# tejeez/sxxcvr

Measured on NVIDIA B200. Metric: rx_unpack+tx_pack throughput, higher is better.
Workload: dtype s32<->f32

## Files before the change

sxxcvr_b200/csrc/sx_kernels.cuh:

```cuda
#pragma once

#include <cuda_runtime.h>
#include <stdint.h>

#include "sx_synth.h"

namespace sx {

template <int WORDS> struct Pack {
    uint32_t w[WORDS];
};

template <int BYTES> __device__ __forceinline__ Pack<BYTES / 4> ld_stream(const void *p);
template <int BYTES> __device__ __forceinline__ void st_stream(void *p, const Pack<BYTES / 4> &v);

template <> __device__ __forceinline__ Pack<1> ld_stream<4>(const void *p)
{
    Pack<1> r;
    asm volatile("ld.global.L1::no_allocate.b32 %0, [%1];" : "=r"(r.w[0]) : "l"(p) : "memory");
    return r;
}
template <> __device__ __forceinline__ Pack<2> ld_stream<8>(const void *p)
{
    Pack<2> r;
    asm volatile("ld.global.L1::no_allocate.v2.b32 {%0,%1}, [%2];"
                 : "=r"(r.w[0]), "=r"(r.w[1])
                 : "l"(p)
                 : "memory");
    return r;
}
template <> __device__ __forceinline__ Pack<4> ld_stream<16>(const void *p)
{
    Pack<4> r;
    asm volatile("ld.global.L1::no_allocate.v4.b32 {%0,%1,%2,%3}, [%4];"
                 : "=r"(r.w[0]), "=r"(r.w[1]), "=r"(r.w[2]), "=r"(r.w[3])
                 : "l"(p)
                 : "memory");
    return r;
}
template <> __device__ __forceinline__ Pack<8> ld_stream<32>(const void *p)
{
    Pack<8> r;
    asm volatile("ld.global.L1::no_allocate.L2::evict_first.v8.b32 {%0,%1,%2,%3,%4,%5,%6,%7}, [%8];"
                 : "=r"(r.w[0]), "=r"(r.w[1]), "=r"(r.w[2]), "=r"(r.w[3]), "=r"(r.w[4]),
                   "=r"(r.w[5]), "=r"(r.w[6]), "=r"(r.w[7])
                 : "l"(p)
                 : "memory");
    return r;
}

template <> __device__ __forceinline__ void st_stream<4>(void *p, const Pack<1> &v)
{
    asm volatile("st.global.L1::no_allocate.b32 [%0], %1;" ::"l"(p), "r"(v.w[0]) : "memory");
}
template <> __device__ __forceinline__ void st_stream<8>(void *p, const Pack<2> &v)
{
    asm volatile("st.global.L1::no_allocate.v2.b32 [%0], {%1,%2};" ::"l"(p), "r"(v.w[0]),
                 "r"(v.w[1])
                 : "memory");
}
template <> __device__ __forceinline__ void st_stream<16>(void *p, const Pack<4> &v)
{
    asm volatile("st.global.L1::no_allocate.v4.b32 [%0], {%1,%2,%3,%4};" ::"l"(p), "r"(v.w[0]),
                 "r"(v.w[1]), "r"(v.w[2]), "r"(v.w[3])
                 : "memory");
}
template <> __device__ __forceinline__ void st_stream<32>(void *p, const Pack<8> &v)
{
    asm volatile("st.global.L1::no_allocate.L2::evict_first.v8.b32 [%0], {%1,%2,%3,%4,%5,%6,%7,%8};" ::"l"(p),
                 "r"(v.w[0]), "r"(v.w[1]), "r"(v.w[2]), "r"(v.w[3]), "r"(v.w[4]), "r"(v.w[5]),
                 "r"(v.w[6]), "r"(v.w[7])
                 : "memory");
}


struct RxCf32 {
    static constexpr int kSrcWords = 2, kDstWords = 2;
    template <int FR>
    __device__ __forceinline__ static void apply(const Pack<2 * FR> &in, Pack<2 * FR> &out, float)
    {
#pragma unroll
        for (int i = 0; i < 2 * FR; i++)
            out.w[i] = __float_as_uint(__int2float_rn(int(in.w[i])) * 4.656612873077392578125e-10f);
    }
};

__device__ __forceinline__ uint32_t tx_component(float f)
{
    return uint32_t(__float2int_rz(f * 2147483648.0f)) & 0xFFFFFFFCu;
}

__device__ __forceinline__ uint32_t tx_enable_bits(float fi, float fq, float thr2)
{
    float mag2 = __fadd_rn(__fmul_rn(fi, fi), __fmul_rn(fq, fq));
    return (mag2 >= thr2) ? 3u : 0u;
}

struct TxCf32 {
    static constexpr int kSrcWords = 2, kDstWords = 2;
    template <int FR>
    __device__ __forceinline__ static void apply(const Pack<2 * FR> &in, Pack<2 * FR> &out,
                                                 float thr2)
    {
#pragma unroll
        for (int n = 0; n < FR; n++) {
            float fi = __uint_as_float(in.w[2 * n]), fq = __uint_as_float(in.w[2 * n + 1]);
            out.w[2 * n] = tx_component(fi) | tx_enable_bits(fi, fq, thr2);
            out.w[2 * n + 1] = tx_component(fq);
        }
    }
};

struct RxCs16 {
    static constexpr int kSrcWords = 2, kDstWords = 1;
    template <int FR>
    __device__ __forceinline__ static void apply(const Pack<2 * FR> &in, Pack<FR> &out, float)
    {
#pragma unroll
        for (int n = 0; n < FR; n++)
            out.w[n] = __byte_perm(in.w[2 * n], in.w[2 * n + 1], 0x7632);
    }
};

struct TxCs16 {
    static constexpr int kSrcWords = 1, kDstWords = 2;
    template <int FR>
    __device__ __forceinline__ static void apply(const Pack<FR> &in, Pack<2 * FR> &out, float thr2)
    {
#pragma unroll
        for (int n = 0; n < FR; n++) {
            uint32_t w = in.w[n];
            float fi = __int2float_rn(int(short(w & 0xFFFFu))) * 3.0517578125e-05f;
            float fq = __int2float_rn(int(w) >> 16) * 3.0517578125e-05f;
            out.w[2 * n] = (w << 16) | tx_enable_bits(fi, fq, thr2);
            out.w[2 * n + 1] = w & 0xFFFF0000u;
        }
    }
};

struct RxS16Cf32 {
    static constexpr int kSrcWords = 1, kDstWords = 2;
    template <int FR>
    __device__ __forceinline__ static void apply(const Pack<FR> &in, Pack<2 * FR> &out, float)
    {
#pragma unroll
        for (int n = 0; n < FR; n++) {
            uint32_t w = in.w[n];
            out.w[2 * n] = __float_as_uint(__int2float_rn(int(short(w & 0xFFFFu))) * 3.0517578125e-05f);
            out.w[2 * n + 1] = __float_as_uint(__int2float_rn(int(w) >> 16) * 3.0517578125e-05f);
        }
    }
};

struct TxCf32S16 {
    static constexpr int kSrcWords = 2, kDstWords = 1;
    __device__ __forceinline__ static uint32_t component(float f)
    {
        int v = __float2int_rz(f * 32768.0f);
        v = v > 32767 ? 32767 : (v < -32768 ? -32768 : v);
        return uint32_t(v) & 0xFFFCu;
    }
    template <int FR>
    __device__ __forceinline__ static void apply(const Pack<2 * FR> &in, Pack<FR> &out, float thr2)
    {
#pragma unroll
        for (int n = 0; n < FR; n++) {
            float fi = __uint_as_float(in.w[2 * n]), fq = __uint_as_float(in.w[2 * n + 1]);
            out.w[n] = (component(fi) | tx_enable_bits(fi, fq, thr2)) | (component(fq) << 16);
        }
    }
};

struct StreamArgs {
    const char *src;
    char *dst;
    uint64_t total;
    uint64_t head;
    uint64_t nvec;
    float thr2;
};

template <class Op, int FR, int UNROLL, int BLOCK>
__global__ void __launch_bounds__(BLOCK) stream_convert_kernel(const StreamArgs a)
{
    constexpr int SB = Op::kSrcWords * 4 * FR, DB = Op::kDstWords * 4 * FR;
    constexpr uint64_t TILE = uint64_t(BLOCK) * UNROLL;
    const char *src = a.src + a.head * (Op::kSrcWords * 4);
    char *dst = a.dst + a.head * (Op::kDstWords * 4);

    for (uint64_t base = uint64_t(blockIdx.x) * TILE; base < a.nvec;
         base += uint64_t(gridDim.x) * TILE) {
        Pack<Op::kSrcWords * FR> in[UNROLL];
        Pack<Op::kDstWords * FR> out[UNROLL];
        const uint64_t first = base + threadIdx.x;
        const char *sp = src + first * SB;
        char *dp = dst + first * DB;
        if (base + TILE <= a.nvec) {
#pragma unroll
            for (int j = 0; j < UNROLL; j++)
                in[j] = ld_stream<SB>(sp + size_t(j) * BLOCK * SB);
#pragma unroll
            for (int j = 0; j < UNROLL; j++)
                Op::template apply<FR>(in[j], out[j], a.thr2);
#pragma unroll
            for (int j = 0; j < UNROLL; j++)
                st_stream<DB>(dp + size_t(j) * BLOCK * DB, out[j]);
        } else {
#pragma unroll
            for (int j = 0; j < UNROLL; j++) {
                if (first + uint64_t(j) * BLOCK < a.nvec) {
                    in[j] = ld_stream<SB>(sp + size_t(j) * BLOCK * SB);
                    Op::template apply<FR>(in[j], out[j], a.thr2);
                    st_stream<DB>(dp + size_t(j) * BLOCK * DB, out[j]);
                }
            }
        }
    }

    if (blockIdx.x == 0) {
        const uint64_t mid = a.nvec * FR;
        const uint64_t nedge = a.total - mid;
        if (threadIdx.x < nedge) {
            uint64_t f = threadIdx.x < a.head ? threadIdx.x : mid + threadIdx.x;
            Pack<Op::kSrcWords> in1 = ld_stream<Op::kSrcWords * 4>(a.src + f * (Op::kSrcWords * 4));
            Pack<Op::kDstWords> out1;
            Op::template apply<1>(in1, out1, a.thr2);
            st_stream<Op::kDstWords * 4>(a.dst + f * (Op::kDstWords * 4), out1);
        }
    }
}

template <class Op>
__global__ void word_convert_kernel(const char *src, char *dst, uint64_t total, float thr2)
{
    for (uint64_t f = uint64_t(blockIdx.x) * blockDim.x + threadIdx.x; f < total;
         f += uint64_t(gridDim.x) * blockDim.x) {
        Pack<Op::kSrcWords> in;
        Pack<Op::kDstWords> out;
#pragma unroll
        for (int i = 0; i < Op::kSrcWords; i++)
            in.w[i] = ld_stream<4>(src + (f * Op::kSrcWords + i) * 4).w[0];
        Op::template apply<1>(in, out, thr2);
#pragma unroll
        for (int i = 0; i < Op::kDstWords; i++) {
            Pack<1> o;
            o.w[0] = out.w[i];
            st_stream<4>(dst + (f * Op::kDstWords + i) * 4, o);
        }
    }
}

namespace bulk {

__device__ __forceinline__ uint32_t smem_u32(const void *p)
{
    return uint32_t(__cvta_generic_to_shared(p));
}
__device__ __forceinline__ void mbar_init(uint64_t *bar, uint32_t count)
{
    asm volatile("mbarrier.init.shared::cta.b64 [%0], %1;" ::"r"(smem_u32(bar)), "r"(count));
}
__device__ __forceinline__ void mbar_expect_tx(uint64_t *bar, uint32_t bytes)
{
    asm volatile("mbarrier.arrive.expect_tx.shared::cta.b64 _, [%0], %1;" ::"r"(smem_u32(bar)),
                 "r"(bytes)
                 : "memory");
}
__device__ __forceinline__ void mbar_wait(uint64_t *bar, uint32_t parity)
{
    asm volatile("{\n"
                 ".reg .pred p;\n"
                 "WAIT_%=:\n"
                 "mbarrier.try_wait.parity.shared::cta.b64 p, [%0], %1;\n"
                 "@p bra DONE_%=;\n"
                 "bra WAIT_%=;\n"
                 "DONE_%=:\n"
                 "}" ::"r"(smem_u32(bar)),
                 "r"(parity)
                 : "memory");
}
__device__ __forceinline__ uint64_t make_policy(int kind)
{
    uint64_t pol;
    switch (kind) {
    case 1: asm volatile("createpolicy.fractional.L2::evict_normal.b64 %0, 1.0;" : "=l"(pol)); break;
    case 2: asm volatile("createpolicy.fractional.L2::evict_last.b64 %0, 1.0;" : "=l"(pol)); break;
    case 3: asm volatile("createpolicy.fractional.L2::evict_unchanged.b64 %0, 1.0;" : "=l"(pol)); break;
    default: asm volatile("createpolicy.fractional.L2::evict_first.b64 %0, 1.0;" : "=l"(pol)); break;
    }
    return pol;
}
__device__ __forceinline__ void load_g2s(void *smem_dst, const void *gsrc, uint32_t bytes,
                                         uint64_t *bar, uint64_t pol)
{
    asm volatile("cp.async.bulk.shared::cluster.global.mbarrier::complete_tx::bytes.L2::cache_hint "
                 "[%0], [%1], %2, [%3], %4;" ::"r"(smem_u32(smem_dst)),
                 "l"(gsrc), "r"(bytes), "r"(smem_u32(bar)), "l"(pol)
                 : "memory");
}
__device__ __forceinline__ void store_s2g(void *gdst, const void *smem_src, uint32_t bytes,
                                          uint64_t pol)
{
    asm volatile("cp.async.bulk.global.shared::cta.bulk_group.L2::cache_hint [%0], [%1], %2, %3;" ::"l"(gdst),
                 "r"(smem_u32(smem_src)), "r"(bytes), "l"(pol)
                 : "memory");
}
__device__ __forceinline__ void commit_group()
{
    asm volatile("cp.async.bulk.commit_group;" ::: "memory");
}
template <int N> __device__ __forceinline__ void wait_group_read()
{
    asm volatile("cp.async.bulk.wait_group.read %0;" ::"n"(N) : "memory");
}
__device__ __forceinline__ void wait_group_all()
{
    asm volatile("cp.async.bulk.wait_group 0;" ::: "memory");
}
__device__ __forceinline__ void fence_async_smem()
{
    asm volatile("fence.proxy.async.shared::cta;" ::: "memory");
}

}

struct BulkArgs {
    const char *src;
    char *dst;
    uint64_t nframes;
    float thr2;
    int load_policy;
    int store_policy;
    int contiguous;
};

template <class Op, int TILE, int STAGES, bool SKEW = false>
__global__ void bulk_convert_kernel(const BulkArgs a)
{
    constexpr int SFB = Op::kSrcWords * 4, DFB = Op::kDstWords * 4;
    static_assert(!SKEW || (SFB == 8 && DFB == 8), "the skewed variant is for 8-byte frames on both sides");
    constexpr int PAD = SKEW ? 16 : 0;
    constexpr size_t IN_STAGE = size_t(TILE) * SFB + PAD;
    extern __shared__ __align__(128) unsigned char smem[];
    unsigned char *in_buf = smem;
    unsigned char *out_buf = smem + size_t(STAGES) * IN_STAGE;
    uint64_t *full = reinterpret_cast<uint64_t *>(out_buf + size_t(STAGES) * TILE * DFB);

    const uint64_t ntiles = (a.nframes + TILE - 1) / TILE;
    uint64_t first, stride, mine;
    if (a.contiguous) {
        const uint64_t per = (ntiles + gridDim.x - 1) / gridDim.x;
        first = uint64_t(blockIdx.x) * per;
        stride = 1;
        mine = first >= ntiles ? 0 : (ntiles - first < per ? ntiles - first : per);
    } else {
        first = blockIdx.x;
        stride = gridDim.x;
        mine = first >= ntiles ? 0 : (ntiles - first + stride - 1) / stride;
    }
    if (mine == 0)
        return;
    const uint64_t pol = bulk::make_policy(a.load_policy), pol_store = bulk::make_policy(a.store_policy);

    auto tile_frames = [&](uint64_t i) -> uint32_t {
        uint64_t t = first + i * stride;
        uint64_t left = a.nframes - t * TILE;
        return uint32_t(left < uint64_t(TILE) ? left : uint64_t(TILE));
    };

    if (threadIdx.x == 0) {
        for (int s = 0; s < STAGES; s++)
            bulk::mbar_init(&full[s], 1);
        asm volatile("fence.mbarrier_init.release.cluster;" ::: "memory");
    }
    __syncthreads();

    if (threadIdx.x == 0) {
        for (uint64_t i = 0; i < uint64_t(STAGES) && i < mine; i++) {
            uint32_t nf = tile_frames(i);
            bulk::mbar_expect_tx(&full[i], nf * SFB + PAD);
            bulk::load_g2s(in_buf + i * IN_STAGE, a.src + (first + i * stride) * TILE * SFB,
                           nf * SFB + PAD, &full[i], pol);
        }
    }

    for (uint64_t i = 0; i < mine; i++) {
        const int s = int(i % STAGES);
        const uint32_t parity = uint32_t(i / STAGES) & 1u;
        const uint32_t nf = tile_frames(i);

        if (threadIdx.x == 0)
            bulk::wait_group_read<STAGES - 1>();
        __syncthreads();

        bulk::mbar_wait(&full[s], parity);

        const unsigned char *ib = in_buf + size_t(s) * IN_STAGE + (SKEW ? 8 : 0);
        unsigned char *ob = out_buf + size_t(s) * TILE * DFB;
        constexpr int FR = (Op::kSrcWords == 1 || Op::kDstWords == 1) ? 4 : 2;
        for (uint32_t v = threadIdx.x; v * FR < nf; v += blockDim.x) {
            Pack<Op::kSrcWords * FR> in;
            Pack<Op::kDstWords * FR> out;
            if constexpr (SKEW) {
                const uint2 *ip = reinterpret_cast<const uint2 *>(ib + size_t(v) * FR * SFB);
#pragma unroll
                for (int q = 0; q < FR; q++) {
                    uint2 t = ip[q];
                    in.w[2 * q] = t.x, in.w[2 * q + 1] = t.y;
                }
            } else {
                const uint4 *ip = reinterpret_cast<const uint4 *>(ib + size_t(v) * FR * SFB);
#pragma unroll
                for (int q = 0; q < Op::kSrcWords * FR / 4; q++) {
                    uint4 t = ip[q];
                    in.w[4 * q] = t.x, in.w[4 * q + 1] = t.y, in.w[4 * q + 2] = t.z, in.w[4 * q + 3] = t.w;
                }
            }
            Op::template apply<FR>(in, out, a.thr2);
            uint4 *op = reinterpret_cast<uint4 *>(ob + size_t(v) * FR * DFB);
#pragma unroll
            for (int q = 0; q < Op::kDstWords * FR / 4; q++)
                op[q] = make_uint4(out.w[4 * q], out.w[4 * q + 1], out.w[4 * q + 2], out.w[4 * q + 3]);
        }
        bulk::fence_async_smem();
        __syncthreads();

        if (threadIdx.x == 0) {
            bulk::store_s2g(a.dst + (first + i * stride) * TILE * DFB, ob, nf * DFB, pol_store);
            bulk::commit_group();
            uint64_t nxt = i + STAGES;
            if (nxt < mine) {
                uint32_t nnf = tile_frames(nxt);
                bulk::mbar_expect_tx(&full[s], nnf * SFB + PAD);
                bulk::load_g2s(in_buf + size_t(s) * IN_STAGE,
                               a.src + (first + nxt * stride) * TILE * SFB, nnf * SFB + PAD, &full[s], pol);
            }
        }
    }
    if (threadIdx.x == 0)
        bulk::wait_group_all();
}

struct LoopbackArgs {
    const char *i2s_in;
    char *cf32;
    char *i2s_out;
    uint64_t nvec;
    uint64_t total;
    float thr2;
};

template <int UNROLL>
__global__ void loopback_kernel(const LoopbackArgs a)
{
    const uint64_t tile = uint64_t(blockDim.x) * UNROLL;
    for (uint64_t base = uint64_t(blockIdx.x) * tile; base < a.nvec;
         base += uint64_t(gridDim.x) * tile) {
        Pack<4> in[UNROLL];
#pragma unroll
        for (int j = 0; j < UNROLL; j++) {
            uint64_t v = base + threadIdx.x + uint64_t(j) * blockDim.x;
            if (v < a.nvec)
                in[j] = ld_stream<16>(a.i2s_in + v * 16);
        }
#pragma unroll
        for (int j = 0; j < UNROLL; j++) {
            uint64_t v = base + threadIdx.x + uint64_t(j) * blockDim.x;
            if (v < a.nvec) {
                Pack<4> mid, out;
                RxCf32::apply<2>(in[j], mid, 0.0f);
                TxCf32::apply<2>(mid, out, a.thr2);
                if (a.cf32)
                    st_stream<16>(a.cf32 + v * 16, mid);
                st_stream<16>(a.i2s_out + v * 16, out);
            }
        }
    }
    if (blockIdx.x == 0 && threadIdx.x == 0 && (a.total & 1)) {
        uint64_t f = a.total - 1;
        Pack<2> in1 = ld_stream<8>(a.i2s_in + f * 8), mid, out;
        RxCf32::apply<1>(in1, mid, 0.0f);
        TxCf32::apply<1>(mid, out, a.thr2);
        if (a.cf32)
            st_stream<8>(a.cf32 + f * 8, mid);
        st_stream<8>(a.i2s_out + f * 8, out);
    }
}

struct BlockDesc {
    const char *src;
    char *dst;
    uint64_t length;
    float thr2;
    uint32_t reserved;
};

template <class Op>
__device__ __forceinline__ void convert_span(const BlockDesc &b, uint64_t lo, uint64_t hi,
                                             uint32_t tid, uint32_t nthreads)
{
    constexpr int SFB = Op::kSrcWords * 4, DFB = Op::kDstWords * 4;
    constexpr int FR = 16 / (SFB < DFB ? SFB : DFB);
    const bool vec_ok = ((reinterpret_cast<uintptr_t>(b.src) + lo * SFB) % (SFB * FR) == 0) &&
                        ((reinterpret_cast<uintptr_t>(b.dst) + lo * DFB) % (DFB * FR) == 0);
    uint64_t done = lo;
    if (vec_ok) {
        uint64_t nvec = (hi - lo) / FR;
        constexpr int U = 4;
        uint64_t v = tid;
        for (; v + uint64_t(U - 1) * nthreads < nvec; v += uint64_t(U) * nthreads) {
            Pack<Op::kSrcWords * FR> in[U];
#pragma unroll
            for (int u = 0; u < U; u++)
                in[u] = ld_stream<SFB * FR>(b.src + (lo + (v + uint64_t(u) * nthreads) * FR) * SFB);
#pragma unroll
            for (int u = 0; u < U; u++) {
// ... 505 lines not shown
```

sxxcvr_b200/csrc/sxgpu.cu:

```cuda
#include "../../include/sxgpu.h"

#include "sx_kernels.cuh"
#include "sx_bank.cuh"
#include "sx_iir.cuh"
#include "sx_resident.cuh"
#include "host/par_copy.hpp"
#include "host/worker_pool.hpp"

#include <algorithm>
#include <atomic>
#include <chrono>
#include <cmath>
#include <cstdio>
#include <cstdlib>
#include <cstring>
#include <map>
#include <memory>
#include <mutex>
#include <string>
#include <tuple>
#include <type_traits>
#include <vector>

#include <sched.h>

using namespace sx;

namespace {

constexpr int kRingSlots = 4;

struct HostRing {
    size_t chunk_frames = 0;
    void *d_in[kRingSlots] = {};
    void *d_out[kRingSlots] = {};
    void *h_in[kRingSlots] = {};
    void *h_out[kRingSlots] = {};
    cudaEvent_t copied_in[kRingSlots] = {};
    cudaEvent_t converted[kRingSlots] = {};
    cudaEvent_t done[kRingSlots] = {};
    bool events = false;
};

struct alignas(64) SmallFlag {
    volatile unsigned long long done;
};

struct HostLane {
    std::mutex mutex;
    cudaStream_t s_h2d = nullptr, s_comp = nullptr, s_d2h = nullptr;
    cudaStream_t s_slot[kRingSlots] = {};
    HostRing ring;
    std::unique_ptr<sxhost::ParallelCopier> copier_in, copier_out;
    sxhost::Sidekick retirer;
    sxhost::Progress issued, retired;
    std::atomic<int> pipeline_error{0};

    SmallFlag *flag = nullptr;
    unsigned int *d_arrivals = nullptr;
    unsigned long long flag_seq = 0;

    Mailbox *mailbox = nullptr;
    cudaStream_t s_resident = nullptr;
    unsigned long long resident_seq = 0;
};

}

struct sxgpu_ctx {
    int device = 0;
    cudaDeviceProp prop;
    cudaStream_t stream = nullptr;

    int64_t rx_variant = 0, tx_variant = 0;
    int64_t unroll = 0;
    int64_t block = 0;
    int64_t ctas_per_sm = 0;
    int64_t bulk_tile = 0, bulk_stages = 0;
    int64_t bulk_load_policy = 0, bulk_store_policy = 0;
    int64_t bulk_contiguous = 0;
    int64_t host_chunk_frames = 0;
    int64_t host_chunk_min_frames = 0;
    int64_t host_mode = 0;
    int64_t small_mode = 0;
    int64_t host_in_mode = 0;
    int64_t host_out_mode = 0;
    int64_t bounce_nt = 1;
    int64_t pipeline_mode = 0;
    int64_t zero_copy_max_frames = 1 << 18;
    int64_t resident_max_frames = 0;
    int64_t zero_copy_variant = 1;
    int64_t batch_variant = 0;
    int64_t loopback_variant = 0;
    int64_t warp_ctas_per_sm = 0;
    int64_t bank_split_variant = 0;
    int64_t bank_pdl = 1;
    int64_t bank_repeat_variant = 0;
    int64_t bounce_threads = 0;
    int64_t numa_local_alloc = 1;
    int64_t numa_node = -1;

    cpu_set_t local_cpus;
    bool have_local_cpus = false;

    std::atomic<uint64_t> resident_launches{0}, resident_calls{0}, flagged_calls{0};
    std::atomic<int> live_banks{0};
    std::atomic<int> live_iirs{0};
    bool l2_carveout_set = false;

    HostLane lanes[2];

    cudaMemPool_t scratch_pool = nullptr;

    StatsAcc *d_stats = nullptr;
    StatsAcc *h_stats = nullptr;
    std::mutex stats_mutex;

    std::atomic<uint64_t> launches{0}, frames_rx{0}, frames_tx{0}, h2d_bytes{0}, d2h_bytes{0};

    std::mutex err_mutex;
    std::string last_error;
    uint64_t error_serial = 0;

    std::mutex occupancy_mutex;
    std::map<std::tuple<const void *, int, size_t>, int> occupancy;

    int fail(cudaError_t e, const char *what)
    {
        std::lock_guard<std::mutex> lock(err_mutex);
        last_error = std::string(what) + ": " + cudaGetErrorString(e);
        error_serial++;
        cudaGetLastError();
        return (e == cudaErrorMemoryAllocation) ? SXGPU_ERR_NOMEM : SXGPU_ERR_CUDA;
    }
    int invalid(const char *what)
    {
        std::lock_guard<std::mutex> lock(err_mutex);
        last_error = what;
        error_serial++;
        return SXGPU_ERR_INVALID;
    }
};

namespace {

void read_gpu_locality(sxgpu_ctx *ctx)
{
    CPU_ZERO(&ctx->local_cpus);
    char bdf[32] = {0};
    if (cudaDeviceGetPCIBusId(bdf, sizeof bdf, ctx->device) != cudaSuccess) {
        cudaGetLastError();
        return;
    }
    for (char *c = bdf; *c; c++)
        if (*c >= 'A' && *c <= 'F')
            *c = char(*c - 'A' + 'a');
    const std::string base = std::string("/sys/bus/pci/devices/") + bdf + "/";
    if (FILE *f = std::fopen((base + "numa_node").c_str(), "r")) {
        long node = -1;
        if (std::fscanf(f, "%ld", &node) == 1)
            ctx->numa_node = node;
        std::fclose(f);
    }
    if (FILE *f = std::fopen((base + "local_cpulist").c_str(), "r")) {
        int lo = 0, hi = 0, count = 0;
        for (;;) {
            if (std::fscanf(f, "%d", &lo) != 1)
                break;
            hi = lo;
            int c = std::fgetc(f);
            if (c == '-') {
                if (std::fscanf(f, "%d", &hi) != 1)
                    break;
                c = std::fgetc(f);
            }
            for (int cpu = lo; cpu <= hi && cpu < CPU_SETSIZE; cpu++, count++)
                CPU_SET(cpu, &ctx->local_cpus);
            if (c != ',')
                break;
        }
        std::fclose(f);
        ctx->have_local_cpus = count > 0;
    }
}

class NearGpu {
public:
    explicit NearGpu(sxgpu_ctx *ctx)
    {
        if (!ctx->numa_local_alloc || !ctx->have_local_cpus)
            return;
        if (sched_getaffinity(0, sizeof saved_, &saved_) != 0)
            return;
        cpu_set_t want;
        CPU_AND(&want, &saved_, &ctx->local_cpus);
        if (CPU_COUNT(&want) == 0 || CPU_EQUAL(&want, &saved_))
            return;
        bound_ = sched_setaffinity(0, sizeof want, &want) == 0;
    }
    ~NearGpu()
    {
        if (bound_)
            sched_setaffinity(0, sizeof saved_, &saved_);
    }
    NearGpu(const NearGpu &) = delete;
    NearGpu &operator=(const NearGpu &) = delete;

private:
    cpu_set_t saved_;
    bool bound_ = false;
};

}

#define SX_CUDA(ctx, call)                                                                     \
    do {                                                                                       \
        cudaError_t e_ = (call);                                                               \
        if (e_ != cudaSuccess)                                                                 \
            return (ctx)->fail(e_, #call);                                                     \
    } while (0)

#define SX_TRY(expr)                                                                           \
    do {                                                                                       \
        int r_ = (expr);                                                                       \
        if (r_ != SXGPU_OK)                                                                    \
            return r_;                                                                         \
    } while (0)

namespace {

typedef void (*StreamKernel)(const StreamArgs);
typedef void (*BulkKernel)(const BulkArgs);

template <class Op, int FR, int BLOCK> StreamKernel stream_kernel_for_unroll(int unroll)
{
    switch (unroll) {
    case 2: return stream_convert_kernel<Op, FR, 2, BLOCK>;
    case 8: return stream_convert_kernel<Op, FR, 8, BLOCK>;
    default: return stream_convert_kernel<Op, FR, 4, BLOCK>;
    }
}

template <class Op> StreamKernel stream_kernel(int fr, int unroll, int block)
{
    if (fr == 4)
        return block == 512 ? stream_kernel_for_unroll<Op, 4, 512>(unroll)
                            : stream_kernel_for_unroll<Op, 4, 256>(unroll);
    if (fr == 2)
        return block == 512 ? stream_kernel_for_unroll<Op, 2, 512>(unroll)
                            : stream_kernel_for_unroll<Op, 2, 256>(unroll);
    return stream_convert_kernel<Op, 1, 4, 256>;
}

struct BulkShape {
    int tile, stages;
};

template <class Op> BulkKernel bulk_kernel(BulkShape s)
{
    if (s.tile == 4096 && s.stages == 3) return bulk_convert_kernel<Op, 4096, 3>;
    if (s.tile == 3072 && s.stages == 4) return bulk_convert_kernel<Op, 3072, 4>;
    if (s.tile == 2048 && s.stages == 6) return bulk_convert_kernel<Op, 2048, 6>;
    if (s.tile == 2048 && s.stages == 5) return bulk_convert_kernel<Op, 2048, 5>;
    if (s.tile == 2048 && s.stages == 4) return bulk_convert_kernel<Op, 2048, 4>;
    if (s.tile == 2048 && s.stages == 3) return bulk_convert_kernel<Op, 2048, 3>;
    if (s.tile == 1024 && s.stages == 6) return bulk_convert_kernel<Op, 1024, 6>;
    if (s.tile == 1024 && s.stages == 4) return bulk_convert_kernel<Op, 1024, 4>;
    if (s.tile == 512 && s.stages == 4) return bulk_convert_kernel<Op, 512, 4>;
    return nullptr;
}

template <class Op> size_t bulk_smem_bytes(BulkShape s, bool skew = false)
{
    return size_t(s.stages) * (size_t(s.tile) * (Op::kSrcWords + Op::kDstWords) * 4 + (skew ? 16 : 0)) +
           size_t(s.stages) * 8;
}

template <class Op> BulkKernel bulk_skew_kernel(BulkShape s)
{
    if constexpr (Op::kSrcWords == 2 && Op::kDstWords == 2) {
        if (s.tile == 2048 && s.stages == 4) return bulk_convert_kernel<Op, 2048, 4, true>;
        if (s.tile == 1024 && s.stages == 4) return bulk_convert_kernel<Op, 1024, 4, true>;
    }
    return nullptr;
}

int normalise_unroll(int64_t u)
{
    return (u == 2 || u == 4 || u == 8) ? int(u) : 4;
}

template <class K>
int persistent_grid(sxgpu_ctx *ctx, K kernel, int block, size_t smem, uint64_t work_items)
{
    int per_sm = int(ctx->ctas_per_sm);
    if (per_sm <= 0) {
        std::lock_guard<std::mutex> lock(ctx->occupancy_mutex);
        auto key = std::make_tuple(reinterpret_cast<const void *>(kernel), block, smem);
        auto it = ctx->occupancy.find(key);
        if (it == ctx->occupancy.end()) {
            int occ = 0;
            if (cudaOccupancyMaxActiveBlocksPerMultiprocessor(&occ, kernel, block, smem) != cudaSuccess ||
                occ <= 0) {
                cudaGetLastError();
                occ = 1;
            }
            it = ctx->occupancy.emplace(key, occ).first;
        }
        per_sm = it->second;
    }
    uint64_t grid = uint64_t(ctx->prop.multiProcessorCount) * uint64_t(per_sm);
    grid = std::min<uint64_t>(grid, std::max<uint64_t>(work_items, 1));
    return int(grid);
}

struct Plan {
    int fr = 0;
    uint64_t head = 0;
};

template <class Op> Plan plan_access(const char *src, const char *dst, uint64_t total, int want_fr)
{
    constexpr uintptr_t SFB = Op::kSrcWords * 4, DFB = Op::kDstWords * 4;
    uintptr_t s = reinterpret_cast<uintptr_t>(src), d = reinterpret_cast<uintptr_t>(dst);
    Plan p;
    if (s % SFB != 0 || d % DFB != 0)
        return p;
    for (int fr = want_fr; fr >= 1; fr >>= 1) {
        uintptr_t a = (s / SFB) % fr, b = (d / DFB) % fr;
        if (a != b)
            continue;
        p.fr = fr;
        p.head = std::min<uint64_t>((fr - a) % fr, total);
        return p;
    }
    p.fr = 1;
    return p;
}

template <class Op>
int launch_bulk(sxgpu_ctx *ctx, const char *src, const char *dst_c, uint64_t total, float thr2,
                cudaStream_t st, bool *handled)
{
    char *dst = const_cast<char *>(dst_c);
    constexpr uintptr_t SFB = Op::kSrcWords * 4, DFB = Op::kDstWords * 4;
    constexpr uint64_t G = 16 / (SFB < DFB ? SFB : DFB);
    *handled = false;

    uint64_t head = 0;
    bool found = false;
    for (; head < G; head++) {
        if ((reinterpret_cast<uintptr_t>(src) + head * SFB) % 16 == 0 &&
            (reinterpret_cast<uintptr_t>(dst) + head * DFB) % 16 == 0) {
            found = true;
            break;
        }
    }

    const int big_tile = (SFB == DFB) ? 2048 : 3072;
    BulkShape shape = {int(ctx->bulk_tile ? ctx->bulk_tile : (total >= (uint64_t(1) << 24) ? big_tile : 1024)),
                       int(ctx->bulk_stages ? ctx->bulk_stages : 4)};
    BulkKernel k = nullptr;
    bool skew = false;
    uint64_t mid = 0;
    if (found) {
        if (total < head + G)
            return SXGPU_OK;
        mid = (total - head) / G * G;
        k = bulk_kernel<Op>(shape);
        if (!k)
            return ctx->invalid("unsupported bulk_tile/bulk_stages combination");
    } else {
        k = bulk_skew_kernel<Op>(shape);
        if (!k || reinterpret_cast<uintptr_t>(src) % 8 || reinterpret_cast<uintptr_t>(dst) % 8)
            return SXGPU_OK;
        head = (reinterpret_cast<uintptr_t>(dst) % 16) ? 1 : 2;
        if (total < head + 3)
            return SXGPU_OK;
        mid = (total - head - 1) / 2 * 2;
        skew = true;
    }
    size_t smem = bulk_smem_bytes<Op>(shape, skew);
    int block = int(ctx->block ? ctx->block : 256);

    BulkArgs a = {src + head * SFB - (skew ? 8 : 0), dst + head * DFB, mid, thr2, int(ctx->bulk_load_policy),
                  int(ctx->bulk_store_policy), int(ctx->bulk_contiguous)};
    uint64_t ntiles = (mid + shape.tile - 1) / shape.tile;
    int grid = persistent_grid(ctx, k, block, smem, ntiles);
    k<<<grid, block, smem, st>>>(a);
    SX_CUDA(ctx, cudaGetLastError());
    ctx->launches++;

    uint64_t tail = total - head - mid;
    if (head) {
        StreamArgs e = {src, dst, head, head, 0, thr2};
        stream_convert_kernel<Op, 1, 4, 256><<<1, 256, 0, st>>>(e);
        SX_CUDA(ctx, cudaGetLastError());
        ctx->launches++;
    }
    if (tail) {
        StreamArgs e = {src + (head + mid) * SFB, dst + (head + mid) * DFB, tail, tail, 0, thr2};
        stream_convert_kernel<Op, 1, 4, 256><<<1, 256, 0, st>>>(e);
        SX_CUDA(ctx, cudaGetLastError());
        ctx->launches++;
    }
    *handled = true;
    return SXGPU_OK;
}

template <class Op>
int launch_convert(sxgpu_ctx *ctx, const void *src_v, void *dst_v, uint64_t total, float thr2,
                   int64_t variant, cudaStream_t st)
{
    if (total == 0)
        return SXGPU_OK;
    const char *src = static_cast<const char *>(src_v);
    char *dst = static_cast<char *>(dst_v);
    if (reinterpret_cast<uintptr_t>(src) % 4 || reinterpret_cast<uintptr_t>(dst) % 4)
        return ctx->invalid("sample buffers must be at least 4-byte aligned");

    if (variant == 0)
        variant = 4;
    if (variant == 4) {
        constexpr bool narrow = Op::kSrcWords != Op::kDstWords;
        Plan p = plan_access<Op>(src, dst, total, narrow ? 4 : 2);
        if (p.fr >= 2 && total >= p.head + uint64_t(p.fr)) {
            constexpr int block = 256;
            const int unroll = total < (uint64_t(1) << 21) ? 4 : 2;
            StreamArgs a = {src, dst, total, p.head, (total - p.head) / uint64_t(p.fr), thr2};
            StreamKernel k = stream_kernel<Op>(p.fr, unroll, block);
            uint64_t tiles = (a.nvec + uint64_t(block) * unroll - 1) / (uint64_t(block) * unroll);
            k<<<unsigned(std::min<uint64_t>(tiles, 0x7fffffffu)), block, 0, st>>>(a);
            SX_CUDA(ctx, cudaGetLastError());
            ctx->launches++;
            return SXGPU_OK;
        }
        variant = 3;
    }
    if (variant == 3) {
        bool handled = false;
        SX_TRY(launch_bulk<Op>(ctx, src, dst, total, thr2, st, &handled));
        if (handled)
            return SXGPU_OK;
        variant = 1;
    }

    Plan p = plan_access<Op>(src, dst, total, variant == 2 ? 4 : 2);
    if (p.fr == 0) {
        const int block = 256;
        uint64_t ctas = (total + block - 1) / block;
        int grid = persistent_grid(ctx, word_convert_kernel<Op>, block, 0, ctas);
        word_convert_kernel<Op><<<grid, block, 0, st>>>(src, dst, total, thr2);
        SX_CUDA(ctx, cudaGetLastError());
        ctx->launches++;
        return SXGPU_OK;
    }

    int unroll = p.fr == 1 ? 4 : normalise_unroll(ctx->unroll);
    int block = (p.fr != 1 && ctx->block == 512) ? 512 : 256;
    StreamArgs a = {src, dst, total, p.head, (total - p.head) / uint64_t(p.fr), thr2};
    StreamKernel k = stream_kernel<Op>(p.fr, unroll, block);
    uint64_t tiles = (a.nvec + uint64_t(block) * unroll - 1) / (uint64_t(block) * unroll);
    int grid = persistent_grid(ctx, k, block, 0, tiles);
    k<<<grid, block, 0, st>>>(a);
    SX_CUDA(ctx, cudaGetLastError());
    ctx->launches++;
    return SXGPU_OK;
}

bool frames_overflow(size_t offset, size_t length)
{
    const size_t cap = size_t(1) << 60;
    return offset > cap || length > cap || offset + length > cap;
}

template <class Op>
int convert_entry(sxgpu_ctx *ctx, const void *d_src, size_t src_offset, void *d_dest,
                  size_t dest_offset, size_t length, float thr2, int64_t variant,
                  sxgpu_stream stream)
{
    if (!ctx)
        return SXGPU_ERR_INVALID;
    if (length == 0)
        return SXGPU_OK;
    if (!d_src || !d_dest)
        return ctx->invalid("null sample buffer");
    if (frames_overflow(src_offset, length) || frames_overflow(dest_offset, length))
        return ctx->invalid("offset + length overflows");
    SX_CUDA(ctx, cudaSetDevice(ctx->device));
    const char *src = static_cast<const char *>(d_src) + src_offset * (Op::kSrcWords * 4);
    char *dst = static_cast<char *>(d_dest) + dest_offset * (Op::kDstWords * 4);
    cudaStream_t st = stream ? static_cast<cudaStream_t>(stream) : ctx->stream;
    return launch_convert<Op>(ctx, src, dst, length, thr2, variant, st);
}

struct HostPtrInfo {
    bool pinned = false;
    bool on_device = false;
    bool foreign_device = false;
    void *device_alias = nullptr;
};

HostPtrInfo classify_pointer(const sxgpu_ctx *ctx, const void *p)
{
    HostPtrInfo info;
    cudaPointerAttributes attr;
    if (cudaPointerGetAttributes(&attr, p) != cudaSuccess) {
        cudaGetLastError();
        return info;
    }
    if (attr.type == cudaMemoryTypeHost) {
        info.pinned = true;
        info.device_alias = attr.devicePointer;
    } else if (attr.type == cudaMemoryTypeDevice || attr.type == cudaMemoryTypeManaged) {
        info.on_device = true;
        info.foreign_device = attr.type == cudaMemoryTypeDevice && attr.device != ctx->device;
        info.device_alias = attr.devicePointer;
    }
    return info;
}

size_t pick_chunk_frames(const sxgpu_ctx *ctx, size_t length)
{
    if (ctx->host_chunk_frames > 0)
        return size_t(std::max<int64_t>(ctx->host_chunk_frames, 1024));
    size_t chunk = size_t(1) << 17;
    while (chunk < (size_t(1) << 22) && chunk * 4 < length)
        chunk <<= 1;
    return chunk;
}

int ensure_lane(sxgpu_ctx *ctx, HostLane &lane)
{
    if (!lane.s_h2d) {
        SX_CUDA(ctx, cudaStreamCreateWithFlags(&lane.s_h2d, cudaStreamDefault));
        SX_CUDA(ctx, cudaStreamCreateWithFlags(&lane.s_comp, cudaStreamDefault));
        SX_CUDA(ctx, cudaStreamCreateWithFlags(&lane.s_d2h, cudaStreamDefault));
        for (int i = 0; i < kRingSlots; i++)
            SX_CUDA(ctx, cudaStreamCreateWithFlags(&lane.s_slot[i], cudaStreamDefault));
    }
    HostRing &r = lane.ring;
    if (!r.events) {
        for (int i = 0; i < kRingSlots; i++) {
            SX_CUDA(ctx, cudaEventCreateWithFlags(&r.copied_in[i], cudaEventDisableTiming));
            SX_CUDA(ctx, cudaEventCreateWithFlags(&r.converted[i], cudaEventDisableTiming));
            SX_CUDA(ctx, cudaEventCreateWithFlags(&r.done[i], cudaEventDisableTiming));
        }
        r.events = true;
    }
    if (!lane.flag) {
        SX_CUDA(ctx, cudaHostAlloc(reinterpret_cast<void **>(&lane.flag), sizeof(SmallFlag),
                                   cudaHostAllocMapped | cudaHostAllocPortable));
        lane.flag->done = 0;
        SX_CUDA(ctx, cudaMalloc(reinterpret_cast<void **>(&lane.d_arrivals), sizeof(unsigned int)));
        SX_CUDA(ctx, cudaMemset(lane.d_arrivals, 0, sizeof(unsigned int)));
    }
    return SXGPU_OK;
}

void resident_stop(sxgpu_ctx *, HostLane &lane)
{
    if (!lane.mailbox || !lane.s_resident)
        return;
    volatile Mailbox *box = lane.mailbox;
    box->quit = 1;
    std::atomic_thread_fence(std::memory_order_seq_cst);
    cudaStreamSynchronize(lane.s_resident);
    box->quit = 0;
}

int ensure_ring(sxgpu_ctx *ctx, HostLane &lane, size_t frames, bool bounce_in, bool bounce_out)
{
    SX_TRY(ensure_lane(ctx, lane));
    HostRing &r = lane.ring;
    if (frames > r.chunk_frames) {
        resident_stop(ctx, lane);
        for (int i = 0; i < kRingSlots; i++) {
            if (r.d_in[i]) cudaFree(r.d_in[i]);
            if (r.d_out[i]) cudaFree(r.d_out[i]);
            if (r.h_in[i]) cudaFreeHost(r.h_in[i]);
            if (r.h_out[i]) cudaFreeHost(r.h_out[i]);
            r.d_in[i] = r.d_out[i] = r.h_in[i] = r.h_out[i] = nullptr;
        }
        r.chunk_frames = 0;
        for (int i = 0; i < kRingSlots; i++) {
            SX_CUDA(ctx, cudaMalloc(&r.d_in[i], frames * 8));
            SX_CUDA(ctx, cudaMalloc(&r.d_out[i], frames * 8));
        }
        r.chunk_frames = frames;
    }
    bool missing = false;
    for (int i = 0; i < kRingSlots; i++)
        missing = missing || (bounce_in && !r.h_in[i]) || (bounce_out && !r.h_out[i]);
    if (!missing)
        return SXGPU_OK;
    NearGpu near(ctx);
    for (int i = 0; i < kRingSlots; i++) {
        if (bounce_in && !r.h_in[i])
            SX_CUDA(ctx, cudaHostAlloc(&r.h_in[i], r.chunk_frames * 8, cudaHostAllocDefault));
        if (bounce_out && !r.h_out[i])
            SX_CUDA(ctx, cudaHostAlloc(&r.h_out[i], r.chunk_frames * 8, cudaHostAllocDefault));
    }
    return SXGPU_OK;
}

int resident_convert_call(sxgpu_ctx *ctx, HostLane &lane, int op, const void *src, void *dst, size_t length,
                          float thr2)
{
    using clock = std::chrono::steady_clock;
    if (!lane.mailbox) {
        SX_CUDA(ctx, cudaHostAlloc(reinterpret_cast<void **>(&lane.mailbox), sizeof(Mailbox),
                                   cudaHostAllocMapped | cudaHostAllocPortable));
        std::memset(lane.mailbox, 0, sizeof(Mailbox));
        SX_CUDA(ctx, cudaStreamCreateWithFlags(&lane.s_resident, cudaStreamNonBlocking));
    }
    volatile Mailbox *box = lane.mailbox;

    auto ensure_listening = [&]() -> int {
        if (box->alive)
            return SXGPU_OK;
        SX_CUDA(ctx, cudaStreamSynchronize(lane.s_resident));
        resident_kernel<<<1, 256, 0, lane.s_resident>>>(lane.mailbox, lane.resident_seq);
        SX_CUDA(ctx, cudaGetLastError());
        ctx->launches++;
        ctx->resident_launches++;
        auto t0 = clock::now();
        while (!box->alive) {
            if (clock::now() - t0 > std::chrono::seconds(2))
                return ctx->invalid("resident converter did not start");
        }
        return SXGPU_OK;
    };
    SX_TRY(ensure_listening());

    const unsigned long long seq = ++lane.resident_seq;
    unsigned thr2_bits;
    std::memcpy(&thr2_bits, &thr2, sizeof thr2_bits);
    box->src = static_cast<const char *>(src);
    box->dst = static_cast<char *>(dst);
    std::atomic_thread_fence(std::memory_order_release);
    box->packed = (unsigned long long)(unsigned(length) | (unsigned(op) << 16) | (unsigned(seq & 0x7FFFu) << 17)) |
                  ((unsigned long long)thr2_bits << 32);
    box->request2 = seq;
    std::atomic_thread_fence(std::memory_order_release);
    box->request = seq;

    auto t0 = clock::now();
    unsigned spins = 0;
    while (box->done != seq) {
        if ((++spins & 0xFF) != 0)
            continue;
        if (!box->alive) {
            SX_CUDA(ctx, cudaStreamSynchronize(lane.s_resident));
            if (box->done == seq)
                break;
            lane.resident_seq = seq - 1;
            SX_TRY(ensure_listening());
            lane.resident_seq = seq;
            t0 = clock::now();
        }
        if (clock::now() - t0 > std::chrono::seconds(2))
            return ctx->invalid("resident converter did not answer");
    }
    std::atomic_thread_fence(std::memory_order_acquire);
    ctx->resident_calls++;
    return SXGPU_OK;
}

template <class Op> constexpr int resident_op()
{
    return -1;
}
template <> constexpr int resident_op<RxCf32>()
{
    return 0;
}
template <> constexpr int resident_op<TxCf32>()
{
    return 1;
}

template <class Op>
int flagged_convert_call(sxgpu_ctx *ctx, HostLane &lane, const void *src, void *dst, size_t length, float thr2)
{
    using clock = std::chrono::steady_clock;
    FlaggedArgs a;
    a.block.src = static_cast<const char *>(src);
    a.block.dst = static_cast<char *>(dst);
    a.block.length = length;
    a.block.thr2 = thr2;
    a.block.reserved = 0;
    a.arrivals = lane.d_arrivals;
    a.h_flag = const_cast<unsigned long long *>(&lane.flag->done);
    a.seq = ++lane.flag_seq;
    const int grid = int(std::min<uint64_t>((length + 1023) / 1024, uint64_t(ctx->prop.multiProcessorCount)));
    flagged_convert_kernel<Op><<<grid, 256, 0, lane.s_comp>>>(a);
    SX_CUDA(ctx, cudaGetLastError());
    ctx->launches++;
    unsigned spins = 0;
    auto t0 = clock::now();
    while (lane.flag->done != a.seq) {
        if ((++spins & 0xFFF) != 0)
            continue;
        cudaError_t q = cudaStreamQuery(lane.s_comp);
        if (q != cudaSuccess && q != cudaErrorNotReady)
            return ctx->fail(q, "small-call kernel");
        if (q == cudaSuccess && lane.flag->done != a.seq && clock::now() - t0 > std::chrono::milliseconds(100))
            return ctx->invalid("small-call kernel finished without raising its flag");
        if (clock::now() - t0 > std::chrono::seconds(5))
            return ctx->invalid("small-call kernel did not finish");
    }
    std::atomic_thread_fence(std::memory_order_acquire);
    ctx->flagged_calls++;
    return SXGPU_OK;
}

unsigned bounce_thread_count(const sxgpu_ctx *ctx)
{
    unsigned threads = unsigned(std::min<int64_t>(ctx->bounce_threads, 64));
    if (threads == 0) {
        static const unsigned automatic = [] {
            unsigned ranks = 1;
            if (const char *env = std::getenv("LOCAL_WORLD_SIZE"))
                ranks = unsigned(std::max(1, std::atoi(env)));
            return std::max(1u, std::min(8u, std::thread::hardware_concurrency() / (2 * ranks)));
        }();
        threads = automatic;
    }
    return threads;
}

void bounce_copy(sxgpu_ctx *ctx, std::unique_ptr<sxhost::ParallelCopier> &copier, void *dst, const void *src,
                 size_t bytes)
{
// ... 1910 lines not shown
```

Before: 426,800.

## Add L2 evict-first hints and rotate tile order for L2 handoff between kernels

Stream conversion kernels now use createpolicy-based L2::evict_first cache hints on loads, and on stores for TX ops. For TX ops, the tile traversal is rotated so the final tiles, sized to about half the L2, are processed first. This likely relies on the preceding RX kernel having left its last-written output in L2, so the TX kernel can read those tiles while they are still resident. The costs are a modulo-style remap per tile and a dependence on L2 size and on the order of back-to-back kernels.

After: 429,000, median of 6. No clear change (+0.5%).

```diff
diff --git a/sxxcvr_b200/csrc/sx_kernels.cuh b/sxxcvr_b200/csrc/sx_kernels.cuh
--- a/sxxcvr_b200/csrc/sx_kernels.cuh
+++ b/sxxcvr_b200/csrc/sx_kernels.cuh
@@ -73,9 +73,67 @@
                  : "memory");
 }
 
+__device__ __forceinline__ uint64_t l2_evict_first_policy()
+{
+    uint64_t pol;
+    asm volatile("createpolicy.fractional.L2::evict_first.b64 %0, 1.0;" : "=l"(pol));
+    return pol;
+}
+template <int BYTES> __device__ __forceinline__ Pack<BYTES / 4> ld_hinted(const void *p, uint64_t pol);
+template <int BYTES> __device__ __forceinline__ void st_hinted(void *p, const Pack<BYTES / 4> &v, uint64_t pol);
+
+template <> __device__ __forceinline__ Pack<2> ld_hinted<8>(const void *p, uint64_t pol)
+{
+    Pack<2> r;
+    asm volatile("ld.global.L1::no_allocate.L2::cache_hint.v2.b32 {%0,%1}, [%2], %3;"
+                 : "=r"(r.w[0]), "=r"(r.w[1])
+                 : "l"(p), "l"(pol)
+                 : "memory");
+    return r;
+}
+template <> __device__ __forceinline__ Pack<4> ld_hinted<16>(const void *p, uint64_t pol)
+{
+    Pack<4> r;
+    asm volatile("ld.global.L1::no_allocate.L2::cache_hint.v4.b32 {%0,%1,%2,%3}, [%4], %5;"
+                 : "=r"(r.w[0]), "=r"(r.w[1]), "=r"(r.w[2]), "=r"(r.w[3])
+                 : "l"(p), "l"(pol)
+                 : "memory");
+    return r;
+}
+template <> __device__ __forceinline__ Pack<8> ld_hinted<32>(const void *p, uint64_t pol)
+{
+    Pack<8> r;
+    asm volatile("ld.global.L1::no_allocate.L2::cache_hint.v8.b32 {%0,%1,%2,%3,%4,%5,%6,%7}, [%8], %9;"
+                 : "=r"(r.w[0]), "=r"(r.w[1]), "=r"(r.w[2]), "=r"(r.w[3]), "=r"(r.w[4]),
+                   "=r"(r.w[5]), "=r"(r.w[6]), "=r"(r.w[7])
+                 : "l"(p), "l"(pol)
+                 : "memory");
+    return r;
+}
+template <> __device__ __forceinline__ void st_hinted<8>(void *p, const Pack<2> &v, uint64_t pol)
+{
+    asm volatile("st.global.L1::no_allocate.L2::cache_hint.v2.b32 [%0], {%1,%2}, %3;" ::"l"(p),
+                 "r"(v.w[0]), "r"(v.w[1]), "l"(pol)
+                 : "memory");
+}
+template <> __device__ __forceinline__ void st_hinted<16>(void *p, const Pack<4> &v, uint64_t pol)
+{
+    asm volatile("st.global.L1::no_allocate.L2::cache_hint.v4.b32 [%0], {%1,%2,%3,%4}, %5;" ::"l"(p),
+                 "r"(v.w[0]), "r"(v.w[1]), "r"(v.w[2]), "r"(v.w[3]), "l"(pol)
+                 : "memory");
+}
+template <> __device__ __forceinline__ void st_hinted<32>(void *p, const Pack<8> &v, uint64_t pol)
+{
+    asm volatile("st.global.L1::no_allocate.L2::cache_hint.v8.b32 [%0], {%1,%2,%3,%4,%5,%6,%7,%8}, %9;" ::"l"(p),
+                 "r"(v.w[0]), "r"(v.w[1]), "r"(v.w[2]), "r"(v.w[3]), "r"(v.w[4]), "r"(v.w[5]),
+                 "r"(v.w[6]), "r"(v.w[7]), "l"(pol)
+                 : "memory");
+}
+
 
 struct RxCf32 {
     static constexpr int kSrcWords = 2, kDstWords = 2;
+    static constexpr bool kToI2s = false;
     template <int FR>
     __device__ __forceinline__ static void apply(const Pack<2 * FR> &in, Pack<2 * FR> &out, float)
     {
@@ -98,6 +156,7 @@
 
 struct TxCf32 {
     static constexpr int kSrcWords = 2, kDstWords = 2;
+    static constexpr bool kToI2s = true;
     template <int FR>
     __device__ __forceinline__ static void apply(const Pack<2 * FR> &in, Pack<2 * FR> &out,
                                                  float thr2)
@@ -113,6 +172,7 @@
 
 struct RxCs16 {
     static constexpr int kSrcWords = 2, kDstWords = 1;
+    static constexpr bool kToI2s = false;
     template <int FR>
     __device__ __forceinline__ static void apply(const Pack<2 * FR> &in, Pack<FR> &out, float)
     {
@@ -124,6 +184,7 @@
 
 struct TxCs16 {
     static constexpr int kSrcWords = 1, kDstWords = 2;
+    static constexpr bool kToI2s = true;
     template <int FR>
     __device__ __forceinline__ static void apply(const Pack<FR> &in, Pack<2 * FR> &out, float thr2)
     {
@@ -140,6 +201,7 @@
 
 struct RxS16Cf32 {
     static constexpr int kSrcWords = 1, kDstWords = 2;
+    static constexpr bool kToI2s = false;
     template <int FR>
     __device__ __forceinline__ static void apply(const Pack<FR> &in, Pack<2 * FR> &out, float)
     {
@@ -154,6 +216,7 @@
 
 struct TxCf32S16 {
     static constexpr int kSrcWords = 2, kDstWords = 1;
+    static constexpr bool kToI2s = true;
     __device__ __forceinline__ static uint32_t component(float f)
     {
         int v = __float2int_rz(f * 32768.0f);
@@ -178,18 +241,37 @@
     uint64_t head;
     uint64_t nvec;
     float thr2;
-};
-
-template <class Op, int FR, int UNROLL, int BLOCK>
+    uint64_t first_tile;
+};
+
+template <class Op, int FR, int UNROLL, int BLOCK, bool HINTED = false>
 __global__ void __launch_bounds__(BLOCK) stream_convert_kernel(const StreamArgs a)
 {
     constexpr int SB = Op::kSrcWords * 4 * FR, DB = Op::kDstWords * 4 * FR;
     constexpr uint64_t TILE = uint64_t(BLOCK) * UNROLL;
     const char *src = a.src + a.head * (Op::kSrcWords * 4);
     char *dst = a.dst + a.head * (Op::kDstWords * 4);
-
-    for (uint64_t base = uint64_t(blockIdx.x) * TILE; base < a.nvec;
-         base += uint64_t(gridDim.x) * TILE) {
+    const uint64_t ntiles = (a.nvec + TILE - 1) / TILE;
+    uint64_t pol = 0;
+    if constexpr (HINTED)
+        pol = l2_evict_first_policy();
+    auto load = [&](const char *p) {
+        if constexpr (HINTED)
+            return ld_hinted<SB>(p, pol);
+        else
+            return ld_stream<SB>(p);
+    };
+    auto store = [&](char *p, const Pack<Op::kDstWords * FR> &v) {
+        if constexpr (HINTED && Op::kToI2s)
+            st_hinted<DB>(p, v, pol);
+        else
+            st_stream<DB>(p, v);
+    };
+
+#pragma unroll 1
+    for (uint64_t t = blockIdx.x; t < ntiles; t += gridDim.x) {
+        const uint64_t r = t + a.first_tile;
+        const uint64_t base = (r < ntiles ? r : r - ntiles) * TILE;
         Pack<Op::kSrcWords * FR> in[UNROLL];
         Pack<Op::kDstWords * FR> out[UNROLL];
         const uint64_t first = base + threadIdx.x;
@@ -198,20 +280,20 @@
         if (base + TILE <= a.nvec) {
 #pragma unroll
             for (int j = 0; j < UNROLL; j++)
-                in[j] = ld_stream<SB>(sp + size_t(j) * BLOCK * SB);
+                in[j] = load(sp + size_t(j) * BLOCK * SB);
 #pragma unroll
             for (int j = 0; j < UNROLL; j++)
                 Op::template apply<FR>(in[j], out[j], a.thr2);
 #pragma unroll
             for (int j = 0; j < UNROLL; j++)
-                st_stream<DB>(dp + size_t(j) * BLOCK * DB, out[j]);
+                store(dp + size_t(j) * BLOCK * DB, out[j]);
         } else {
 #pragma unroll
             for (int j = 0; j < UNROLL; j++) {
                 if (first + uint64_t(j) * BLOCK < a.nvec) {
-                    in[j] = ld_stream<SB>(sp + size_t(j) * BLOCK * SB);
+                    in[j] = load(sp + size_t(j) * BLOCK * SB);
                     Op::template apply<FR>(in[j], out[j], a.thr2);
-                    st_stream<DB>(dp + size_t(j) * BLOCK * DB, out[j]);
+                    store(dp + size_t(j) * BLOCK * DB, out[j]);
                 }
             }
         }
diff --git a/sxxcvr_b200/csrc/sxgpu.cu b/sxxcvr_b200/csrc/sxgpu.cu
--- a/sxxcvr_b200/csrc/sxgpu.cu
+++ b/sxxcvr_b200/csrc/sxgpu.cu
@@ -252,6 +252,13 @@
     return stream_convert_kernel<Op, 1, 4, 256>;
 }
 
+template <class Op> StreamKernel direct_kernel(int fr, int unroll)
+{
+    if (fr == 4)
+        return unroll == 4 ? stream_convert_kernel<Op, 4, 4, 256, true> : stream_convert_kernel<Op, 4, 2, 256, true>;
+    return unroll == 4 ? stream_convert_kernel<Op, 2, 4, 256, true> : stream_convert_kernel<Op, 2, 2, 256, true>;
+}
+
 struct BulkShape {
     int tile, stages;
 };
@@ -283,6 +290,11 @@
         if (s.tile == 1024 && s.stages == 4) return bulk_convert_kernel<Op, 1024, 4, true>;
     }
     return nullptr;
+}
+
+uint64_t l2_handoff_tiles(const sxgpu_ctx *ctx, uint64_t tile_src_bytes)
+{
+    return uint64_t(ctx->prop.l2CacheSize) / 2 / tile_src_bytes;
 }
 
 int normalise_unroll(int64_t u)
@@ -427,9 +439,15 @@
         if (p.fr >= 2 && total >= p.head + uint64_t(p.fr)) {
             constexpr int block = 256;
             const int unroll = total < (uint64_t(1) << 21) ? 4 : 2;
-            StreamArgs a = {src, dst, total, p.head, (total - p.head) / uint64_t(p.fr), thr2};
-            StreamKernel k = stream_kernel<Op>(p.fr, unroll, block);
+            StreamArgs a = {src, dst, total, p.head, (total - p.head) / uint64_t(p.fr), thr2, 0};
+            StreamKernel k = direct_kernel<Op>(p.fr, unroll);
             uint64_t tiles = (a.nvec + uint64_t(block) * unroll - 1) / (uint64_t(block) * unroll);
+            if constexpr (Op::kToI2s) {
+                const uint64_t tile_bytes = uint64_t(block) * unroll * p.fr * (Op::kSrcWords * 4);
+                const uint64_t window = l2_handoff_tiles(ctx, tile_bytes);
+                if (tiles > window)
+                    a.first_tile = tiles - window;
+            }
             k<<<unsigned(std::min<uint64_t>(tiles, 0x7fffffffu)), block, 0, st>>>(a);
             SX_CUDA(ctx, cudaGetLastError());
             ctx->launches++;
```
